# se-hwan/landing-controller

Hardware: AMD Instinct MI355X
Metric: landing NLPs solved/sec (SRBM, N=40, batch) (higher is better)
Workload: dtype f64

## Files before the change

### landing-controller_amd/csrc/solver_capi.inc

```

namespace {

struct StageTab {
  std::vector<int> tg_ab, tg_start, tg_term, gm_start, gm_term, a_term, r_start, r_term;
  int nu;
  std::vector<std::array<int, 4>> cterm;
  std::vector<std::array<int, 4>> rterm;
  std::vector<unsigned long long> cloc;
  bool operator==(const StageTab& o) const {
    return nu == o.nu && tg_ab == o.tg_ab && tg_start == o.tg_start && tg_term == o.tg_term && gm_start == o.gm_start &&
           gm_term == o.gm_term && a_term == o.a_term && r_start == o.r_start && r_term == o.r_term && cloc == o.cloc;
  }
};

int w_index(const Layout& L, int k, long long c) {
  const int N = L.N;
  if (c >= L.x_X(k) && c < L.x_X(k) + 12) return (int)(c - L.x_X(k));
  if (c >= L.x_U(k) && c < L.x_U(k) + 24) { const int j = (int)(c - L.x_U(k)); return j < 12 ? 12 + j : 24 + (j - 12); }
  if (k < N - 1 && c >= L.x_U(k + 1) && c < L.x_U(k + 1) + 12) return 36 + (int)(c - L.x_U(k + 1));
  return -1;
}
int jpos(const Layout& L, int k, long long c, long long idx) {
  if (c >= L.x_X(k) && c < L.x_X(k) + 12) return landing::NZ_JX + (int)(idx - L.jx(k));
  if (c >= L.x_U(k) && c < L.x_U(k) + 24) return landing::NZ_JU + (int)(idx - L.ju(k));
// ... 353 lines not shown
  if (!(o.theta_mu > 0.0)) o.theta_mu = ctx->L.run_cost ? 1.5 : 1.8;
  if (!(o.mu_init > 0.0)) o.mu_init = ctx->L.run_cost ? 0.1 : 0.5;
  if (!(o.bound_push > 0.0)) o.bound_push = ctx->L.run_cost ? 0.5 : 1.0;
  std::lock_guard<std::mutex> lock(ctx->mu);
  const int rc = ctx->ws.ensure(ctx->L, B, (hipStream_t)stream);
  if (rc) return fail(rc <= -100 ? LANDING_E_HIP : LANDING_E_ARG, "landing_solve_batch: workspace/table setup failed (" + std::to_string(rc) + ")");
  landing::SolveArgs A;
  A.L = ctx->L; A.B = B; A.o = o; A.p = d_p; A.x0 = d_x0; A.x_out = d_x; A.f_out = d_f; A.lam_out = d_lam_g;
  A.status = d_status; A.iters = d_iters; A.kkt = d_kkt; A.ws = ctx->ws.buf.get(); A.ws_stride = landing::member_stride(ctx->L);
  A.ctab = ctx->ws.d_ctab.get(); A.ctype = ctx->ws.d_ctype.get(); A.c_ml = ctx->ws.c_ml; A.c_mid = ctx->ws.c_mid; A.ccomb = ctx->ws.d_ccomb.get();
  A.rterm = (const unsigned long long*)ctx->ws.d_rterm.get(); A.rlen = ctx->ws.rlen;
  A.prof = ctx->d_prof;
  A.edge_map = ctx->d_edge_map.get();
  A.order = nullptr;
  if (o.dispatch_order && B > 512 && B <= 16384) {
    hipLaunchKernelGGL(landing::landing_order_kernel, dim3((B + 255) / 256), dim3(256), 0, (hipStream_t)stream, ctx->L, B, d_p, ctx->ws.d_order.get());
    A.order = ctx->ws.d_order.get();
  }
  hipLaunchKernelGGL(landing::landing_ipm_kernel, dim3(B), dim3(landing::SOLVER_THREADS), 0, (hipStream_t)stream, A);
  HIP_TRY(hipGetLastError());
  HIP_TRY(hipEventRecord(ctx->ws.done, (hipStream_t)stream));
  return 0;
}

int landing_set_profile_buffer(landing_ctx* ctx, double* d_prof) {
  if (!ctx) return fail(LANDING_E_ARG, "landing_set_profile_buffer: bad argument");
  ctx->d_prof = d_prof;
  return 0;
}

int landing_solve_batch_host(landing_ctx* ctx, int B, const double* p, const double* x0, const landing_solver_opts* opts,
// ... 516 lines not shown
```

### landing-controller_amd/csrc/solver_kernels.hip

```cpp
#include <hip/hip_runtime.h>
#include <math.h>

#include "../../include/landing_nlp.h"
#include "ipm_core.hpp"


namespace landing {

constexpr int NZ_JX = 0, NZ_JU = 157, NZ_JUN = 385, NZ_HX = 613, NZ_HU = 642, NZ_HUN = 802, NZ_TOT = 962;
constexpr int GS = 49;
constexpr int PS = 25;
constexpr int YS = 37;
constexpr int RIC_K = 0, RIC_KAP = 576, RIC_MT = 600, RIC_MV = 888, RIC_PX = 900, RIC_PV = 1188, RIC_STRIDE = 1200;
constexpr int RIC_FWD0 = 288, RIC_FWDN = 612;
constexpr int FILT_CAP = 64;
constexpr int SOLVER_NMAX = 96;
constexpr int ES = 26;
constexpr int SOLVER_THREADS = 256;
constexpr int COND_GAM = 480, COND_AH = 528, COND_STRIDE = 704;
constexpr int RCG = 36;
constexpr int RUNC = 48;

constexpr int CTAB_MLMAX = 6;
__host__ __device__ inline unsigned long long cterm_pack(int sa, int oa, int sb, int ob, bool has_b, int rowq, int rtype, int dst, bool closes) {
  const int nz[7] = {NZ_JX, NZ_JU, NZ_JUN, NZ_HX, NZ_HU, NZ_HUN, NZ_TOT};
  const unsigned pa = (unsigned)(nz[sa] + oa), pb = (unsigned)(nz[sb] + ob);
  const unsigned lo = pa | (pb << 11) | ((unsigned)(has_b ? 1 : 0) << 22) | ((unsigned)rowq << 23) | ((unsigned)rtype << 30);
  const unsigned hi = (unsigned)dst | ((unsigned)(closes ? 1 : 0) << 10);
  return (unsigned long long)lo | ((unsigned long long)hi << 32);
}
__host__ __device__ inline bool cterm_closes(unsigned long long t) { return ((t >> 42) & 1ull) != 0; }
constexpr int CX_SR = NZ_TOT + 48, CX_ONE = CX_SR + 208, CX_MONE = CX_ONE + 1, CX_ZERO = CX_ONE + 2, CX_LEN = CX_ONE + 3;
constexpr int ATAB_TB = 6, ATAB_LTMAX = 6;
constexpr int ASM_NSLOT = 512;

inline size_t member_stride(const Layout& L) {
  return (size_t)4 * L.nx + (size_t)14 * L.ng + L.nnz_jac + L.nnz_hess + (size_t)L.N * RUNC + (size_t)(L.N + 1) * RIC_STRIDE + (size_t)L.N * RCG;
}

enum { PH_EVAL = 0, PH_ERR, PH_SIGRHO, PH_BACK, PH_FWD, PH_DUAL, PH_LS, PH_ACCEPT, PH_NFACT, PH_NTRIAL, PH_NITER, PH_NSTAGE_OK, PH_B_ASM, PH_NSTAGE, PH_B_ELIM, PH_B_POST,
       PH_COUNT = 16 };
#define PROF_ADD(slot, tstart) do { if (SH.prof_on) { const long long n_ = (long long)wall_clock64(); if (threadIdx.x == 0) { SH.prof[slot] += (double)(n_ - (tstart)); (tstart) = n_; } } } while (0)

struct SolveArgs {
  Layout L; int B; landing_solver_opts o; double* prof;
  const double* p; const double* x0;
  double* x_out; double* f_out; double* lam_out; int* status; int* iters; double* kkt;
  double* ws; size_t ws_stride;
  const unsigned long long* rterm; int rlen;
  const unsigned long long* ctab; const int* ctype; int c_ml, c_mid;
  const unsigned long long* ccomb;
  const int* edge_map;
  const int* order;
};

struct MemberMem {
  double *x, *xt, *dx, *gx;
  double *g, *gt, *s, *ds, *zL, *zU, *y, *yn, *sig, *rho;
  double *J, *H, *Hc, *ric, *cond;
  double *en, *ep, *wn, *wp;
};

__device__ __forceinline__ MemberMem carve(const Layout& L, double* w) {
  MemberMem M;
  M.x = w; w += L.nx; M.xt = w; w += L.nx; M.dx = w; w += L.nx; M.gx = w; w += L.nx;
  M.g = w; w += L.ng; M.gt = w; w += L.ng; M.s = w; w += L.ng; M.ds = w; w += L.ng;
  M.zL = w; w += L.ng; M.zU = w; w += L.ng;
  M.y = w; w += L.ng; M.yn = w; w += L.ng;
  M.sig = w; w += L.ng; M.rho = w; w += L.ng;
  M.J = w; w += L.nnz_jac; M.H = w; w += L.nnz_hess; M.Hc = w; w += (size_t)L.N * RUNC; M.ric = w; w += (size_t)(L.N + 1) * RIC_STRIDE; M.cond = w; w += (size_t)L.N * RCG;
  M.en = w; w += L.ng; M.ep = w; w += L.ng; M.wn = w; w += L.ng; M.wp = w;
  return M;
}


constexpr int FWD_DXL_NMAX = 64;
constexpr int XCH = 112 * 4;
static_assert(2 * XCH >= 24 * YS, "A1 also holds Y (24 x YS)");
struct Lds {
  double G[48 * GS];
  double P[24 * PS];
  double A1[2 * XCH];
  double Ah[2 * 12 * YS];
  double gam[48], pv[24], q[24], bv[2 * 12], sig[24], w[48], dinv[24];
  double red[(SOLVER_THREADS / 64) * 6];
  double filt_th[FILT_CAP], filt_ph[FILT_CAP];
  double prof[32];
  int flag;
  int segb[SOLVER_NMAX * 8];
  double carry[ASM_NSLOT];
  double rcl[RCG];
  double jhl[CX_LEN];
  double dump[64];
  const unsigned long long* ctab; const unsigned long long* ccomb; int c_ml, c_mid, rc_on;
  double bnd_lb[36 + 2 * 104], bnd_ub[36 + 2 * 104];
  MemberMem M; Layout L; const double* p; int prof_on;
  IpmCtl ks;
  int clip_now, jamrun, action, fact_failed;
  unsigned long long atab_mid[ATAB_LTMAX * SOLVER_THREADS];
  unsigned long long acomb_mid[SOLVER_THREADS];
};
__shared__ Lds SH;
static_assert(36 * FWD_DXL_NMAX + 12 <= 24 * PS + 2 * XCH + 2 * 12 * YS && offsetof(Lds, A1) == offsetof(Lds, P) + sizeof(double) * 24 * PS && offsetof(Lds, Ah) == offsetof(Lds, A1) + sizeof(double) * 2 * XCH,
              "dx (x layout, N <= FWD_DXL_NMAX) fits the adjacent arrays [P | A1 | A^] (forward_pass / row_products)");
static_assert(offsetof(Lds, atab_mid) <= 65528, "the assembly tables address G, A^, gamma, cx, the partial sums and the dump slots with 16-bit byte offsets");
__host__ __device__ inline unsigned long long aterm_pack(int pa, int pb, int pc, int d, bool keep, bool ah) {
  const unsigned lo = (unsigned)pa | ((unsigned)pb << 16);
  const unsigned hi = (unsigned)pc | (((unsigned)d | (keep ? 1u : 0u) | (ah ? 2u : 0u)) << 16);
  return (unsigned long long)lo | ((unsigned long long)hi << 32);
}
__host__ __device__ inline unsigned long long acomb_pack(int n, int s0, int d, bool ah) {
  return (unsigned long long)((unsigned)n | ((unsigned)s0 << 16)) | ((unsigned long long)((unsigned)d | (ah ? 2u : 0u)) << 32);
}

template <int KT, class FA, class FB>
__device__ __forceinline__ f64x4 mfma_tile(f64x4 c, FA fa, FB fb) {
  const int l = threadIdx.x & 63, ij = l & 15, kq = l >> 4;
// ... 333 lines not shown
template <int NU>
__device__ __forceinline__ bool riccati_step(double* rec, double delta, int k) {
  const bool ok = block_eliminate<NU>(rec, delta, k);
  __syncthreads();
  return ok;
}

__device__ __noinline__ bool riccati_backward(double delta) {
  Lds& S = SH;
  const Layout& L = S.L;
  const MemberMem& M = S.M;
  const double* p = S.p;
  const int N = L.N, lane = threadIdx.x, NT = blockDim.x;
  (void)p; (void)N; (void)lane; (void)NT;
  bool ok = true;
  for (int e = lane; e < 24 * PS; e += NT) S.P[e] = 0.0;
  __syncthreads();
  if (lane < 12) {
    const int i = lane;
    const int ra = i < 6 ? 12 + i : 24 + (i - 6), rb = i < 6 ? 18 + i : 30 + (i - 6);
    const double qn2 = S.ks.feas ? 0.0 : 2.0 * p[L.o_QN + i];
    S.P[i * PS + i] = qn2 + M.sig[ra] + M.sig[rb] + delta;
    S.pv[i] = qn2 * (M.x[12 * N + i] - p[12 * N + i]) + M.rho[ra] + M.rho[rb];
    double* rec = M.ric + (size_t)N * RIC_STRIDE;
    for (int j = 0; j < 24; ++j) rec[RIC_PX + i * 24 + j] = (j == i) ? S.P[i * PS + i] : 0.0;
    rec[RIC_PV + i] = S.pv[i];
  }
  for (int e = lane; e < 48 * GS; e += NT) S.G[e] = 0.0;
  for (int e = lane; e < 2 * 12 * YS; e += NT) S.Ah[e] = 0.0;
  if (lane < 24) S.pv[lane] = (lane < 12) ? S.pv[lane] : 0.0;
// ... 1 lines not shown
  {
    AsmRegs first;
    asm_issue(N - 1, first);
    asm_copy(first);
    __syncthreads();
    asm_terms(N - 1, (N - 1) & 1, first);
    __syncthreads();
    asm_combine(N - 1, (N - 1) & 1);
  }
  __syncthreads();
  for (int k = N - 1; k >= 0 && ok; --k) {
    const bool last = (k == N - 1);
    long long tb_ = S.prof_on ? (long long)wall_clock64() : 0;
    double* rec = M.ric + (size_t)k * RIC_STRIDE;
    ok = last ? riccati_step<12>(rec, delta, k) : riccati_step<24>(rec, delta, k);
    if (lane == 0) { S.prof[PH_NSTAGE] += 1.0; if (ok) S.prof[PH_NSTAGE_OK] += 1.0; }
    PROF_ADD(PH_B_ELIM, tb_);
  }
  if (ok) {
    if (lane < 12) {
      const int i = lane;
      const double x0i = (i < 6) ? p[L.o_q_init + i] : p[L.o_qd_init + i - 6];
      S.sig[i] = x0i - M.x[i];
    }
    for (int e = lane; e < 144; e += NT) { const int i = e / 12, j = e % 12; S.G[(24 + i) * GS + 24 + j] = S.P[(12 + i) * PS + 12 + j]; }
    __syncthreads();
    if (lane < 12) {
      double v = S.pv[12 + lane];
      for (int t = 0; t < 12; ++t) v += S.P[(12 + lane) * PS + t] * S.sig[t];
      S.gam[24 + lane] = v;
    }
    __syncthreads();
    if (lane < 64) gauss_jordan_wave<12>(S.G, S.gam, S.A1, S.A1 + 24 * 24, &S.flag);
    __syncthreads();
    ok = S.flag != 0;
    if (lane == 0) { S.prof[PH_NSTAGE] += 1.0; if (ok) S.prof[PH_NSTAGE_OK] += 1.0; }
    if (ok) {
      if (lane < 12) S.sig[12 + lane] = -S.A1[24 * 24 + lane];
      __syncthreads();
    }
  }
  __syncthreads();
  return ok;
}

__device__ __noinline__ void forward_pass() {
  Lds& S = SH;
  const Layout& L = S.L;
  const MemberMem& M = S.M;
  const int N = L.N, tid = threadIdx.x, NT = blockDim.x;
  double* sg = S.G;
  double* buf = S.jhl;
  double* buf1 = S.A1;
  static_assert(24 * (SOLVER_NMAX + 1) <= 48 * GS && RIC_FWDN <= NZ_TOT + RUNC && RIC_FWDN <= XCH * 2, "forward scratch fits");
  auto slot = [&](int k) { return (k & 1) ? buf1 : buf; };
  auto fetch = [&](int k, double (&r)[3]) {
// ... 155 lines not shown
__global__ void landing_mpc_shift_kernel(Layout L, int B, const double* __restrict__ x_prev, const double* __restrict__ state,
                                         double* __restrict__ p, double* __restrict__ x0) {
  const size_t idx = (size_t)blockIdx.x * blockDim.x + threadIdx.x;
  if (idx >= (size_t)B * L.nx) return;
  const int m = (int)(idx / L.nx), i = (int)(idx % L.nx), N = L.N, nX = 12 * (N + 1);
  const double* xp = x_prev + (size_t)m * L.nx;
  double v;
  if (i < 12) v = state[(size_t)m * 12 + i];
  else if (i < nX) { const int k = i / 12, r = i % 12; v = xp[12 * (k < N ? k + 1 : N) + r]; }
  else { const int j = i - nX, k = j / 24, r = j % 24; v = xp[nX + 24 * (k < N - 1 ? k + 1 : N - 1) + r]; }
  x0[idx] = v;
  if (i < 6) p[(size_t)m * L.np + L.o_q_init + i] = v;
  else if (i < 12) p[(size_t)m * L.np + L.o_qd_init + (i - 6)] = v;
}

__global__ void landing_order_kernel(Layout L, int B, const double* __restrict__ p, int* __restrict__ order) {
  const int m = blockIdx.x * blockDim.x + threadIdx.x;
  if (m >= B) return;
  const int off = L.o_q_init + 2;
  double key = p[(size_t)m * L.np + off];
  if (!(key == key)) key = -INFINITY;
  int rank = 0;
  for (int j = 0; j < B; ++j) {
    double kj = p[(size_t)j * L.np + off];
    if (!(kj == kj)) kj = -INFINITY;
    rank += (kj > key) || (kj == key && j < m);
  }
  order[rank] = m;
}

__global__ void __launch_bounds__(SOLVER_THREADS, SOLVER_MIN_WAVES) landing_ipm_kernel(SolveArgs A) {
  if ((int)blockIdx.x >= A.B) return;
  const int m = A.order ? A.order[blockIdx.x] : (int)blockIdx.x;
  const Layout& L = A.L;
  const int N = L.N, lane = threadIdx.x, NT = blockDim.x;
  const int nx = L.nx, ng = L.ng;
  const double* p = A.p + (size_t)m * L.np;
  const landing_solver_opts& o = A.o;
  const MemberMem M = carve(L, A.ws + (size_t)m * A.ws_stride);
  Lds& S = SH;
  const double INF = INFINITY;
  auto bidx = [N](int r) { if (r < 36) return r; const int k = (r - 36) / 104, q = (r - 36) - 104 * k; return 36 + (k == N - 1 ? 104 : 0) + q; };
  double* __restrict__ r_g = M.g; double* __restrict__ r_gt = M.gt; double* __restrict__ r_s = M.s; double* __restrict__ r_ds = M.ds;
  double* __restrict__ r_zL = M.zL; double* __restrict__ r_zU = M.zU;
  double* __restrict__ r_y = M.y; double* __restrict__ r_yn = M.yn; double* __restrict__ r_sig = M.sig; double* __restrict__ r_rho = M.rho;
  S.M = M; S.L = L; S.p = p; S.prof_on = A.prof != nullptr;
  S.ctab = A.ctab; S.ccomb = A.ccomb; S.c_ml = A.c_ml; S.c_mid = A.c_mid; S.rc_on = 0;
  if (lane < SOLVER_THREADS) S.acomb_mid[lane] = A.ccomb[A.c_mid * SOLVER_THREADS + lane];
  for (int e = lane; e < 64; e += NT) S.dump[e] = 0.0;
  for (int e = lane; e < A.c_ml * SOLVER_THREADS; e += NT) S.atab_mid[e] = A.ctab[(size_t)A.c_mid * A.c_ml * SOLVER_THREADS + e];
  if (lane == 0) { S.jhl[CX_ONE] = 1.0; S.jhl[CX_MONE] = -1.0; S.jhl[CX_ZERO] = 0.0; }
  if (lane < 32) S.prof[lane] = 0.0;
  {
    const int nj = L.nnz_jac, nh = L.nnz_hess;
    for (int k = lane; k < N; k += NT) {
      int* sb = S.segb + k * 8;
      sb[0] = L.jx(k); sb[1] = L.ju(k); sb[2] = k < N - 1 ? L.ju(k + 1) : 0;
      sb[3] = nj + L.hx(k); sb[4] = nj + L.hu(k); sb[5] = k < N - 1 ? nj + L.hu(k + 1) : 0;
      sb[6] = nj + nh + k * RUNC; sb[7] = A.ctype[k];
    }
  }
  __syncthreads();

  for (int i = lane; i < nx; i += NT) {
    double v = A.x0[(size_t)m * nx + i];
    if (i < 6) v = p[L.o_q_init + i]; else if (i < 12) v = p[L.o_qd_init + i - 6];
    M.x[i] = v;
  }
  for (int e = lane; e < 36 + 2 * 104; e += NT) {
    const int r = e < 36 ? e : (e < 36 + 104 ? L.g_stage(0) + (e - 36) : L.g_stage(N - 1) + (e - 36 - 104));
    double lb = 0.0, ub = 0.0;
    if (r < ng) bound_of(L, p, r, lb, ub);
    S.bnd_lb[e] = lb; S.bnd_ub[e] = ub;
  }
  __syncthreads();
  if (L.run_cost) rc_init_hc();
  __syncthreads();
  member_eval_g_rare(L, M.x, p, M.g);
  __syncthreads();
  auto init_slacks = [&](bool back, double mu_) {
    for (int r = lane; r < ng; r += NT) { const double lb = S.bnd_lb[bidx(r)], ub = S.bnd_ub[bidx(r)]; ipm_init_row(M, r, r >= 12 && lb != ub, lb, ub, o, back, mu_); }
    __syncthreads();
  };
  init_slacks(false, 0.0);
  IpmCtl& K = S.ks;
#define KS_BEGIN() __syncthreads(); if (lane == 0) {
#define KS_BEGIN_SYNCED() if (lane == 0) {
#define KS_END() } __syncthreads()
  constexpr int RB = 4;
  auto feas_point_pass = [&](double mu_) {
    ElAcc e{};
    for (int r = lane; r < ng; r += NT) {
      double sg = 0.0, rh = 0.0;
      if (r >= 12) el_point_row(e, M, r, S.bnd_lb[bidx(r)], S.bnd_ub[bidx(r)], mu_, o.feas_rho, sg, rh);
      r_sig[r] = sg; r_rho[r] = rh;
    }
    el_point_finish(K, e, S.red);
  };
  auto point_pass = [&](double mu_) {
    if (K.feas) { feas_point_pass(mu_); return; }
    double pr = 0.0, co = 0.0, cm = 0.0, ys = 0.0, zs = 0.0, nz = 0.0;
    for (int rb = lane; rb < ng; rb += NT * RB) {
      double lbv[RB], ubv[RB], gv[RB], sv[RB], zlv[RB], zuv[RB], yv[RB];
#pragma unroll
      for (int j = 0; j < RB; ++j) { const int r = rb + j * NT, rr = r < ng ? r : ng - 1; lbv[j] = S.bnd_lb[bidx(rr)]; ubv[j] = S.bnd_ub[bidx(rr)]; gv[j] = r_g[rr]; sv[j] = r_s[rr]; zlv[j] = r_zL[rr]; zuv[j] = r_zU[rr]; yv[j] = r_y[rr]; }
#pragma unroll
      for (int j = 0; j < RB; ++j) {
        const int r = rb + j * NT;
        if (r >= ng) continue;
        const double lb = lbv[j], ub = ubv[j];
        double sg = 0.0, rh = 0.0;
        if (r >= 12) {
          const double g = gv[j];
          ys += fabs(yv[j]);
          if (lb == ub) pr = fmax(pr, fabs(g - lb));
// ... 4 lines not shown
            if (ub < INF) { const double d = ub - s, rd = fast_rcp(d), zu = zuv[j]; co = fmax(co, d * zu); cm = fmax(cm, fabs(d * zu - mu_)); sg += zu * rd; rh += mu_ * rd; zs += zu; nz += 1.0; }
            rh += sg * (g - s);
          }
        }
        r_sig[r] = sg; r_rho[r] = rh;
      }
    }
    double v[6] = {pr, co, cm, ys, zs, nz}; const int op[6] = {RMAX, RMAX, RMAX, RSUM, RSUM, RSUM};
    block_reduce<6>(v, op, S.red);
    KS_BEGIN_SYNCED() K.c_pr = v[0]; K.c_co = v[1]; K.c_cm = v[2]; K.c_ys = v[3]; K.c_zs = v[4]; K.c_nz = fmax(v[5], 1.0); KS_END();
  };

  if (lane == 0) {
    ipm_init(K, o);
    K.tp = A.prof ? (long long)wall_clock64() : 0;
    S.clip_now = 0; S.jamrun = 0; S.fact_failed = 0;
  }
  __syncthreads();
  const int nst = N > 36 ? N : 36;

  for (;;) {
    if (A.prof && lane == 0) K.tp = (long long)wall_clock64();
    if ((lane & 63) < nst) member_eval_jh(L, M.x, p, M.y, M.J, M.H, M.gx, nullptr, nullptr, K.feas ? 0.0 : 1.0);
    __syncthreads();
    if (L.run_cost && !K.feas) { rc_add_grad(); __syncthreads(); }
    PROF_ADD(PH_EVAL, K.tp);
    if (K.it == 0) point_pass(K.mu);
    {
      double du = 0.0;
      for (int i = lane + 12; i < nx; i += NT) du = fmax(du, fabs(M.gx[i]));
      du = block_reduce1(du, RMAX, S.red);
      KS_BEGIN_SYNCED()
        ipm_errors(K, o, du);
        S.action = ipm_decide(K, o, S.fact_failed != 0);
        S.fact_failed = 0;
      KS_END();
// ... 64 lines not shown
      if (!K.flag) break;
    }
    if (!K.fact_ok) {
      KS_BEGIN() K.status = K.stalled ? LANDING_STALLED : LANDING_NUMERICAL; S.fact_failed = (o.feas_phase && !K.feas_used && !K.feas) ? 1 : 0; KS_END();
      if (S.fact_failed) continue;
      break;
    }
    KS_BEGIN() ipm_commit_delta(K, o, 0.0); KS_END();
    PROF_ADD(PH_BACK, K.tp);

    forward_pass();
    row_products(A.rterm, A.rlen);

    PROF_ADD(PH_FWD, K.tp);
    {
      const double mu = K.mu;
      const bool feas = K.feas != 0;
      const bool clip_now = !feas && K.clip_k_cur > 1 && (K.c_pr > o.clip_until || (o.jam_clip > 0 && S.jamrun >= o.jam_clip));
      double top[4] = {0.0, 0.0, 0.0, 0.0};
      double m_pr = 0.0, m_du = 0.0, th0 = 0.0, bar = 0.0, dphi = 0.0;
      double f0 = 0.0;
      if (feas) {
        const double frho = o.feas_rho;
        for (int r = lane + 12; r < ng; r += NT) {
          const double lb = S.bnd_lb[bidx(r)], ub = S.bnd_ub[bidx(r)], g = r_g[r];
          if (lb == ub) { th0 += fabs(g - lb); continue; }
          const double s = r_s[r];
          double ds = r_ds[r];
          if (r >= 36) { ds = ds + (g - s); r_ds[r] = ds; }
          th0 += fabs(g - s);
// ... 51 lines not shown
      block_reduce<6>(v, op, S.red);
      if (clip_now) block_top4(top, S.red);
      KS_BEGIN_SYNCED()
        const double tau = K.tau;
        double a_pr = (v[0] > tau) ? tau / v[0] : 1.0;
        K.a_du = (v[1] > tau) ? tau / v[1] : 1.0;
        if (clip_now) {
          const double rk = top[(K.clip_k_cur > 4 ? 4 : K.clip_k_cur) - 1];
          a_pr = (rk > tau) ? tau / rk : 1.0;
        }
        K.a_pr = a_pr;
        S.clip_now = clip_now ? 1 : 0; K.omt = clip_now ? 1.0 - tau : -1.0;
        K.th0 = v[2]; K.dphi = v[4]; K.ph0 = v[5] + mu * v[3];
        if (K.th_max == 0.0) K.th_max = 1e4 * fmax(1.0, v[2]);
        K.alpha = a_pr; K.s_corr = 0.0; K.accepted = 0; K.armijo_step = 0; K.ls_done = a_pr > 1e-10 ? 0 : 1;
      KS_END();
    }
    PROF_ADD(PH_DUAL, K.tp);
    while (!K.ls_done) {
      const double alpha = K.alpha, omt = K.omt, mu = K.mu;
      if (lane == 0) S.prof[PH_NTRIAL] += 1.0;
      for (int i = lane; i < nx; i += NT) M.xt[i] = M.x[i] + alpha * M.dx[i];
      __syncthreads();
      if (lane < nst) member_eval_g(L, M.xt, p, M.gt);
      __syncthreads();
      double tht = 0.0, bt = 0.0, ft = 0.0;
      const bool feas = K.feas != 0;
      if (feas) {
        const double frho = o.feas_rho;
        for (int r = lane + 12; r < ng; r += NT) {
          const double lb = S.bnd_lb[bidx(r)], ub = S.bnd_ub[bidx(r)], g = r_gt[r];
          if (lb == ub) { tht += fabs(g - lb); continue; }
          const double s0 = r_s[r], ds = r_ds[r], s = s0 + alpha * ds;
          tht += fabs(g - s);
          if (lb > -INF) { const double n0 = M.en[r]; const ElStep e = el_step(1.0, s0 - lb + n0, n0, r_zL[r], M.wn[r], mu, frho, ds); const double n = n0 + alpha * e.dn; bt -= log((s - lb + n) * n); ft += frho * n; }
          if (ub < INF) { const double q0 = M.ep[r]; const ElStep e = el_step(-1.0, ub + q0 - s0, q0, r_zU[r], M.wp[r], mu, frho, ds); const double q = q0 + alpha * e.dn; bt -= log((ub + q - s) * q); ft += frho * q; }
        }
      } else
      for (int rb = lane + 12; rb < ng; rb += NT * RB) {
        double lbv[RB], ubv[RB], gv[RB], sv[RB], dsv[RB];
#pragma unroll
        for (int j = 0; j < RB; ++j) { const int r = rb + j * NT, rr = r < ng ? r : ng - 1; lbv[j] = S.bnd_lb[bidx(rr)]; ubv[j] = S.bnd_ub[bidx(rr)]; gv[j] = r_gt[rr]; sv[j] = r_s[rr]; dsv[j] = r_ds[rr]; }
#pragma unroll
        for (int j = 0; j < RB; ++j) {
          if (rb + j * NT >= ng) continue;
          const double lb = lbv[j], ub = ubv[j], g = gv[j];
          if (lb == ub) { tht += fabs(g - lb); continue; }
          double s = sv[j] + alpha * dsv[j];
          if (omt > 0.0) { if (lb > -INF) s = fmax(s, fma(omt, sv[j] - lb, lb)); if (ub < INF) s = fmin(s, fma(-omt, ub - sv[j], ub)); }
          tht += fabs(g - s);
          bt -= log((lb > -INF ? s - lb : 1.0) * (ub < INF ? ub - s : 1.0));
        }
      }
      if (lane < 12 && !feas) { const double d = M.xt[12 * N + lane] - p[12 * N + lane]; ft = p[L.o_QN + lane] * d * d; }
      if (L.run_cost && !feas) ft += rc_f(M.xt);
      { double v[3] = {tht, bt, ft}; const int op[3] = {RSUM, RSUM, RSUM}; block_reduce<3>(v, op, S.red); tht = v[0]; bt = v[1]; ft = v[2]; }
      KS_BEGIN_SYNCED() ipm_ls_test(K, o, tht, ft, bt, S.filt_th, S.filt_ph); KS_END();
      if (K.need_corr) {
        double tht2 = 0.0, bt2 = 0.0;
        for (int rb = lane + 12; rb < ng; rb += NT * RB) {
          double lbv[RB], ubv[RB], gv[RB], sv[RB], dsv[RB];
#pragma unroll
          for (int j = 0; j < RB; ++j) { const int r = rb + j * NT, rr = r < ng ? r : ng - 1; lbv[j] = S.bnd_lb[bidx(rr)]; ubv[j] = S.bnd_ub[bidx(rr)]; gv[j] = r_gt[rr]; sv[j] = r_s[rr]; dsv[j] = r_ds[rr]; }
#pragma unroll
          for (int j = 0; j < RB; ++j) {
            if (rb + j * NT >= ng) continue;
            const double lb = lbv[j], ub = ubv[j], g = gv[j];
            if (lb == ub) { tht2 += fabs(g - lb); continue; }
            double s = sv[j] + alpha * dsv[j];
            if (omt > 0.0) { if (lb > -INF) s = fmax(s, fma(omt, sv[j] - lb, lb)); if (ub < INF) s = fmin(s, fma(-omt, ub - sv[j], ub)); }
            const double lo = lb > -INF ? lb + o.slack_corr * (s - lb) : -INF, hi = ub < INF ? ub - o.slack_corr * (ub - s) : INF;
            s = fmin(fmax(g, lo), hi);
            tht2 += fabs(g - s);
            bt2 -= log((lb > -INF ? s - lb : 1.0) * (ub < INF ? ub - s : 1.0));
          }
        }
        { double v[2] = {tht2, bt2}; const int op[2] = {RSUM, RSUM}; block_reduce<2>(v, op, S.red); tht2 = v[0]; bt2 = v[1]; }
        KS_BEGIN_SYNCED() ipm_ls_corr_test(K, o, tht2, bt2, S.filt_th, S.filt_ph); KS_END();
      }
    }
    KS_BEGIN()
      ipm_ls_end(K, o, S.filt_th, S.filt_ph, FILT_CAP);
      if (o.jam_clip > 0) S.jamrun = (!S.clip_now && K.a_pr < 0.02) ? S.jamrun + 1 : 0;
    KS_END();
    if (K.fallback) {
      const double alpha = K.alpha;
      for (int i = lane; i < nx; i += NT) M.xt[i] = M.x[i] + alpha * M.dx[i];
      __syncthreads();
      member_eval_g_rare(L, M.xt, p, M.gt);
      __syncthreads();
    }
    PROF_ADD(PH_LS, K.tp);
    for (int i = lane; i < nx; i += NT) M.x[i] = M.xt[i];
    if (K.feas) {
      const double alpha = K.alpha, a_du = K.a_du, mu = K.mu, frho = o.feas_rho;
      for (int r = lane; r < ng; r += NT) {
        const double lb = S.bnd_lb[bidx(r)], ub = S.bnd_ub[bidx(r)];
        r_g[r] = r_gt[r];
        if (r < 12) continue;
// ... 6 lines not shown
          const double n = n0 + alpha * e.dn, a = s - lb + n;
          zl = fmin(fmax(z0 + a_du * e.dz, 1e-10 * mu / a), 1e10 * mu / a);
          M.wn[r] = fmin(fmax(w0 + a_du * e.dw, 1e-10 * mu / n), 1e10 * mu / n); M.en[r] = n;
        }
        if (ub < INF) {
          const double q0 = M.ep[r], z0 = r_zU[r], w0 = M.wp[r];
          const ElStep e = el_step(-1.0, ub + q0 - s0, q0, z0, w0, mu, frho, ds);
          const double q = q0 + alpha * e.dn, b = ub + q - s;
          zu = fmin(fmax(z0 + a_du * e.dz, 1e-10 * mu / b), 1e10 * mu / b);
          M.wp[r] = fmin(fmax(w0 + a_du * e.dw, 1e-10 * mu / q), 1e10 * mu / q); M.ep[r] = q;
        }
        r_s[r] = s; r_zL[r] = zl; r_zU[r] = zu; r_y[r] = zu - zl;
      }
      __syncthreads();
      feas_point_pass(mu);
      KS_BEGIN() K.it++; KS_END();
    } else {
      const double alpha = K.alpha, a_du = K.a_du, omt = K.omt, mu = K.mu, s_corr = K.s_corr;
      double npr = 0.0, nco = 0.0, ncm = 0.0, nys = 0.0, nzs = 0.0, nnz = 0.0;
      for (int rb = lane; rb < ng; rb += NT * RB) {
        double lbv[RB], ubv[RB], gv[RB], sv[RB], dsv[RB], zlv[RB], zuv[RB], yv[RB], ynv[RB];
#pragma unroll
        for (int j = 0; j < RB; ++j) {
          const int r = rb + j * NT, rr = r < ng ? r : ng - 1;
          lbv[j] = S.bnd_lb[bidx(rr)]; ubv[j] = S.bnd_ub[bidx(rr)]; gv[j] = r_gt[rr]; sv[j] = r_s[rr]; dsv[j] = r_ds[rr]; zlv[j] = r_zL[rr]; zuv[j] = r_zU[rr]; yv[j] = r_y[rr]; ynv[j] = r_yn[rr];
        }
#pragma unroll
        for (int j = 0; j < RB; ++j) {
          const int r = rb + j * NT;
          if (r >= ng) continue;
          const double lb = lbv[j], ub = ubv[j], g = gv[j];
// ... 21 lines not shown
                nco = fmax(nco, d * zu); ncm = fmax(ncm, fabs(d * zu - mu)); sg += zu * rd; rh += mu * rd; nzs += zu; nnz += 1.0;
              }
              npr = fmax(npr, fabs(g - s));
              rh += sg * (g - s);
              r_s[r] = s; r_zL[r] = zl; r_zU[r] = zu; r_y[r] = zu - zl; nys += fabs(zu - zl);
            }
          }
          r_sig[r] = sg; r_rho[r] = rh;
        }
      }
      double v[6] = {npr, nco, ncm, nys, nzs, nnz}; const int op[6] = {RMAX, RMAX, RMAX, RSUM, RSUM, RSUM};
      block_reduce<6>(v, op, S.red);
      KS_BEGIN_SYNCED()
        K.c_pr = v[0]; K.c_co = v[1]; K.c_cm = v[2]; K.c_ys = v[3]; K.c_zs = v[4]; K.c_nz = fmax(v[5], 1.0);
        K.it++;
      KS_END();
    }
    PROF_ADD(PH_ACCEPT, K.tp);
  }
  __syncthreads();
  if (A.prof && lane == 0) { S.prof[PH_NITER] = (double)K.it; for (int i = 0; i < PH_COUNT; ++i) A.prof[(size_t)m * PH_COUNT + i] = S.prof[i]; }

  double fo = 0.0;
  if (lane < 12) { M.y[lane] = -M.gx[lane]; const double d = M.x[12 * N + lane] - p[12 * N + lane]; fo = p[L.o_QN + lane] * d * d; }
  if (L.run_cost) fo += rc_f(M.x);
  fo = block_reduce1(fo, RSUM, S.red);
  double kp = 0.0, kc = 0.0;
  for (int r = lane; r < ng; r += NT) {
    const double lb = S.bnd_lb[bidx(r)], ub = S.bnd_ub[bidx(r)], g = M.g[r], lam = M.y[r];
    kp = fmax(kp, fmax(lb - g, fmax(g - ub, 0.0)));
    if (lb != ub) {
      const double dist = lam > 0.0 ? ub - g : g - lb;
      if (lam != 0.0 && dist < INF) kc = fmax(kc, fabs(lam * dist));
    }
  }
  { double v[2] = {kp, kc}; const int op[2] = {RMAX, RMAX}; block_reduce<2>(v, op, S.red); kp = v[0]; kc = v[1]; }
  for (int i = lane; i < nx; i += NT) A.x_out[(size_t)m * nx + i] = M.x[i];
  if (A.lam_out) for (int r = lane; r < ng; r += NT) A.lam_out[(size_t)m * ng + r] = M.y[r];
  if (lane == 0) {
    if (A.f_out) A.f_out[m] = fo;
    if (A.status) A.status[m] = K.status;
    if (A.iters) A.iters[m] = K.it;
    if (A.kkt) { A.kkt[3 * m] = kp; A.kkt[3 * m + 1] = K.e_du; A.kkt[3 * m + 2] = kc; }
  }
#undef KS_BEGIN
#undef KS_BEGIN_SYNCED
#undef KS_END
}

}
```

Measured before the change: 19910.

## Fuse first line-search trial with acceptance pass via double-buffered row arrays

On the first line-search trial of a non-feasibility iteration, the kernel now computes the accepted slacks, duals, sigma and rho into a second set of row buffers together with the trial merit terms. It folds the convergence norms into a single 9-value block reduction. When the trial is accepted, pointers are swapped (including x/xt and g/gt) and the separate acceptance pass is skipped, removing a full row sweep and its barriers. In exchange it adds six more per-row workspace arrays, per-phase pointer reloads from shared memory via readfirstlane, and extra work when the first trial is rejected. It also rewrites the order kernel to stage keys through shared memory in tiles and batches the profiling counters for stage attempts.

```diff
diff --git a/landing-controller_amd/csrc/solver_capi.inc b/landing-controller_amd/csrc/solver_capi.inc
--- a/landing-controller_amd/csrc/solver_capi.inc
+++ b/landing-controller_amd/csrc/solver_capi.inc
@@ -391,7 +391,7 @@
   A.edge_map = ctx->d_edge_map.get();
   A.order = nullptr;
   if (o.dispatch_order && B > 512 && B <= 16384) {
-    hipLaunchKernelGGL(landing::landing_order_kernel, dim3((B + 255) / 256), dim3(256), 0, (hipStream_t)stream, ctx->L, B, d_p, ctx->ws.d_order.get());
+    hipLaunchKernelGGL(landing::landing_order_kernel, dim3((B + landing::ORDER_THREADS - 1) / landing::ORDER_THREADS), dim3(landing::ORDER_THREADS), 0, (hipStream_t)stream, ctx->L, B, d_p, ctx->ws.d_order.get());
     A.order = ctx->ws.d_order.get();
   }
   hipLaunchKernelGGL(landing::landing_ipm_kernel, dim3(B), dim3(landing::SOLVER_THREADS), 0, (hipStream_t)stream, A);
diff --git a/landing-controller_amd/csrc/solver_kernels.hip b/landing-controller_amd/csrc/solver_kernels.hip
--- a/landing-controller_amd/csrc/solver_kernels.hip
+++ b/landing-controller_amd/csrc/solver_kernels.hip
@@ -1,5 +1,6 @@
 #include <hip/hip_runtime.h>
 #include <math.h>
+#include <type_traits>
 
 #include "../../include/landing_nlp.h"
 #include "ipm_core.hpp"
@@ -35,12 +36,30 @@
 constexpr int ASM_NSLOT = 512;
 
 inline size_t member_stride(const Layout& L) {
-  return (size_t)4 * L.nx + (size_t)14 * L.ng + L.nnz_jac + L.nnz_hess + (size_t)L.N * RUNC + (size_t)(L.N + 1) * RIC_STRIDE + (size_t)L.N * RCG;
+  return (size_t)4 * L.nx + (size_t)20 * L.ng + L.nnz_jac + L.nnz_hess + (size_t)L.N * RUNC + (size_t)(L.N + 1) * RIC_STRIDE + (size_t)L.N * RCG;
 }
 
 enum { PH_EVAL = 0, PH_ERR, PH_SIGRHO, PH_BACK, PH_FWD, PH_DUAL, PH_LS, PH_ACCEPT, PH_NFACT, PH_NTRIAL, PH_NITER, PH_NSTAGE_OK, PH_B_ASM, PH_NSTAGE, PH_B_ELIM, PH_B_POST,
        PH_COUNT = 16 };
 #define PROF_ADD(slot, tstart) do { if (SH.prof_on) { const long long n_ = (long long)wall_clock64(); if (threadIdx.x == 0) { SH.prof[slot] += (double)(n_ - (tstart)); (tstart) = n_; } } } while (0)
+
+enum { EMU_ACC_FAST = 0, EMU_ACC_FAST_CLIP, EMU_ACC_FIRST_REJECTED, EMU_ACC_BACKTRACK, EMU_ACC_CORR, EMU_ACC_FALLBACK, EMU_ACC_FEAS, EMU_ACC_N };
+#ifndef __HIPCC__
+constexpr int EMU_ACC_MAXB = 64;
+static int emu_acc[EMU_ACC_MAXB][EMU_ACC_N];
+#define LANDING_EMU_COUNT(m, what) do { if ((m) < EMU_ACC_MAXB) emu_acc[m][what]++; } while (0)
+static int emu_fused_on = 1;
+#define LANDING_EMU_FUSED_ON (emu_fused_on != 0)
+extern "C" void landing_emu_set_fused(int on) { emu_fused_on = on; }
+extern "C" int landing_emu_accept_counts(int m, int* counts) {
+  if (m < 0 || m >= EMU_ACC_MAXB || !counts) return -1;
+  for (int i = 0; i < EMU_ACC_N; ++i) counts[i] = emu_acc[m][i];
+  return 0;
+}
+#else
+#define LANDING_EMU_COUNT(m, what) ((void)0)
+#define LANDING_EMU_FUSED_ON true
+#endif
 
 struct SolveArgs {
   Layout L; int B; landing_solver_opts o; double* prof;
@@ -59,7 +78,11 @@
   double *g, *gt, *s, *ds, *zL, *zU, *y, *yn, *sig, *rho;
   double *J, *H, *Hc, *ric, *cond;
   double *en, *ep, *wn, *wp;
+  double *sig2, *rho2, *s2, *zL2, *zU2, *y2;
 };
+constexpr int MEMBER_MEM_PTRS = 29;
+static_assert(sizeof(MemberMem) == MEMBER_MEM_PTRS * sizeof(double*) && std::is_standard_layout<MemberMem>::value && std::is_trivially_copyable<MemberMem>::value,
+              "live_mem() walks MemberMem as an array of double*: nothing but double* members");
 
 __device__ __forceinline__ MemberMem carve(const Layout& L, double* w) {
   MemberMem M;
@@ -69,8 +92,18 @@
   M.y = w; w += L.ng; M.yn = w; w += L.ng;
   M.sig = w; w += L.ng; M.rho = w; w += L.ng;
   M.J = w; w += L.nnz_jac; M.H = w; w += L.nnz_hess; M.Hc = w; w += (size_t)L.N * RUNC; M.ric = w; w += (size_t)(L.N + 1) * RIC_STRIDE; M.cond = w; w += (size_t)L.N * RCG;
-  M.en = w; w += L.ng; M.ep = w; w += L.ng; M.wn = w; w += L.ng; M.wp = w;
+  M.en = w; w += L.ng; M.ep = w; w += L.ng; M.wn = w; w += L.ng; M.wp = w; w += L.ng;
+  M.sig2 = w; w += L.ng; M.rho2 = w; w += L.ng;
+  M.s2 = w; w += L.ng; M.zL2 = w; w += L.ng; M.zU2 = w; w += L.ng; M.y2 = w;
   return M;
+}
+
+__host__ __device__ __forceinline__ void mem_accept_swap(MemberMem& M) {
+  double* t;
+#define LANDING_SWAP(a, b) t = M.a; M.a = M.b; M.b = t
+  LANDING_SWAP(s, s2); LANDING_SWAP(zL, zL2); LANDING_SWAP(zU, zU2); LANDING_SWAP(y, y2); LANDING_SWAP(sig, sig2); LANDING_SWAP(rho, rho2);
+  LANDING_SWAP(g, gt); LANDING_SWAP(x, xt);
+#undef LANDING_SWAP
 }
 
 
@@ -83,7 +116,7 @@
   double A1[2 * XCH];
   double Ah[2 * 12 * YS];
   double gam[48], pv[24], q[24], bv[2 * 12], sig[24], w[48], dinv[24];
-  double red[(SOLVER_THREADS / 64) * 6];
+  double red[(SOLVER_THREADS / 64) * 9];
   double filt_th[FILT_CAP], filt_ph[FILT_CAP];
   double prof[32];
   int flag;
@@ -97,10 +130,25 @@
   MemberMem M; Layout L; const double* p; int prof_on;
   IpmCtl ks;
   int clip_now, jamrun, action, fact_failed;
+  int first_trial, fast;
+  double nxt[6];
   unsigned long long atab_mid[ATAB_LTMAX * SOLVER_THREADS];
   unsigned long long acomb_mid[SOLVER_THREADS];
 };
 __shared__ Lds SH;
+__device__ __forceinline__ MemberMem live_mem() {
+  MemberMem M = SH.M;
+#if defined(__HIP_DEVICE_COMPILE__)
+  double** q = reinterpret_cast<double**>(&M);
+#pragma unroll
+  for (int i = 0; i < MEMBER_MEM_PTRS; ++i) {
+    const unsigned long long a = (unsigned long long)q[i];
+    const unsigned lo = (unsigned)__builtin_amdgcn_readfirstlane((int)(unsigned)a), hi = (unsigned)__builtin_amdgcn_readfirstlane((int)(unsigned)(a >> 32));
+    q[i] = (double*)((unsigned long long)lo | ((unsigned long long)hi << 32));
+  }
+#endif
+  return M;
+}
 static_assert(36 * FWD_DXL_NMAX + 12 <= 24 * PS + 2 * XCH + 2 * 12 * YS && offsetof(Lds, A1) == offsetof(Lds, P) + sizeof(double) * 24 * PS && offsetof(Lds, Ah) == offsetof(Lds, A1) + sizeof(double) * 2 * XCH,
               "dx (x layout, N <= FWD_DXL_NMAX) fits the adjacent arrays [P | A1 | A^] (forward_pass / row_products)");
 static_assert(offsetof(Lds, atab_mid) <= 65528, "the assembly tables address G, A^, gamma, cx, the partial sums and the dump slots with 16-bit byte offsets");
@@ -464,6 +512,7 @@
   const int N = L.N, lane = threadIdx.x, NT = blockDim.x;
   (void)p; (void)N; (void)lane; (void)NT;
   bool ok = true;
+  int n_try = 0;
   for (int e = lane; e < 24 * PS; e += NT) S.P[e] = 0.0;
   __syncthreads();
   if (lane < 12) {
@@ -495,7 +544,7 @@
     long long tb_ = S.prof_on ? (long long)wall_clock64() : 0;
     double* rec = M.ric + (size_t)k * RIC_STRIDE;
     ok = last ? riccati_step<12>(rec, delta, k) : riccati_step<24>(rec, delta, k);
-    if (lane == 0) { S.prof[PH_NSTAGE] += 1.0; if (ok) S.prof[PH_NSTAGE_OK] += 1.0; }
+    ++n_try;
     PROF_ADD(PH_B_ELIM, tb_);
   }
   if (ok) {
@@ -515,12 +564,13 @@
     if (lane < 64) gauss_jordan_wave<12>(S.G, S.gam, S.A1, S.A1 + 24 * 24, &S.flag);
     __syncthreads();
     ok = S.flag != 0;
-    if (lane == 0) { S.prof[PH_NSTAGE] += 1.0; if (ok) S.prof[PH_NSTAGE_OK] += 1.0; }
+    ++n_try;
     if (ok) {
       if (lane < 12) S.sig[12 + lane] = -S.A1[24 * 24 + lane];
       __syncthreads();
     }
   }
+  if (lane == 0) { S.prof[PH_NSTAGE] += (double)n_try; S.prof[PH_NSTAGE_OK] += (double)(ok ? n_try : n_try - 1); }
   __syncthreads();
   return ok;
 }
@@ -706,19 +756,24 @@
   else if (i < 12) p[(size_t)m * L.np + L.o_qd_init + (i - 6)] = v;
 }
 
-__global__ void landing_order_kernel(Layout L, int B, const double* __restrict__ p, int* __restrict__ order) {
-  const int m = blockIdx.x * blockDim.x + threadIdx.x;
-  if (m >= B) return;
+constexpr int ORDER_THREADS = 256;
+__global__ void __launch_bounds__(ORDER_THREADS) landing_order_kernel(Layout L, int B, const double* __restrict__ p, int* __restrict__ order) {
+  __shared__ double keys[ORDER_THREADS];
+  const int tid = threadIdx.x, m = blockIdx.x * ORDER_THREADS + tid;
   const int off = L.o_q_init + 2;
-  double key = p[(size_t)m * L.np + off];
+  double key = m < B ? p[(size_t)m * L.np + off] : 0.0;
   if (!(key == key)) key = -INFINITY;
   int rank = 0;
-  for (int j = 0; j < B; ++j) {
-    double kj = p[(size_t)j * L.np + off];
+  for (int j0 = 0; j0 < B; j0 += ORDER_THREADS) {
+    double kj = j0 + tid < B ? p[(size_t)(j0 + tid) * L.np + off] : 0.0;
     if (!(kj == kj)) kj = -INFINITY;
-    rank += (kj > key) || (kj == key && j < m);
-  }
-  order[rank] = m;
+    keys[tid] = kj;
+    __syncthreads();
+    const int n = B - j0 < ORDER_THREADS ? B - j0 : ORDER_THREADS;
+    for (int j = 0; j < n; ++j) rank += (keys[j] > key) || (keys[j] == key && j0 + j < m);
+    __syncthreads();
+  }
+  if (m < B) order[rank] = m;
 }
 
 __global__ void __launch_bounds__(SOLVER_THREADS, SOLVER_MIN_WAVES) landing_ipm_kernel(SolveArgs A) {
@@ -733,9 +788,10 @@
   Lds& S = SH;
   const double INF = INFINITY;
   auto bidx = [N](int r) { if (r < 36) return r; const int k = (r - 36) / 104, q = (r - 36) - 104 * k; return 36 + (k == N - 1 ? 104 : 0) + q; };
-  double* __restrict__ r_g = M.g; double* __restrict__ r_gt = M.gt; double* __restrict__ r_s = M.s; double* __restrict__ r_ds = M.ds;
-  double* __restrict__ r_zL = M.zL; double* __restrict__ r_zU = M.zU;
-  double* __restrict__ r_y = M.y; double* __restrict__ r_yn = M.yn; double* __restrict__ r_sig = M.sig; double* __restrict__ r_rho = M.rho;
+#define ROW_PTRS(M) double* __restrict__ r_g = (M).g; double* __restrict__ r_gt = (M).gt; double* __restrict__ r_s = (M).s; double* __restrict__ r_ds = (M).ds; \
+  double* __restrict__ r_zL = (M).zL; double* __restrict__ r_zU = (M).zU; double* __restrict__ r_y = (M).y; double* __restrict__ r_yn = (M).yn; \
+  double* __restrict__ r_sig = (M).sig; double* __restrict__ r_rho = (M).rho; \
+  (void)r_g; (void)r_gt; (void)r_s; (void)r_ds; (void)r_zL; (void)r_zU; (void)r_y; (void)r_yn; (void)r_sig; (void)r_rho
   S.M = M; S.L = L; S.p = p; S.prof_on = A.prof != nullptr;
   S.ctab = A.ctab; S.ccomb = A.ccomb; S.c_ml = A.c_ml; S.c_mid = A.c_mid; S.rc_on = 0;
   if (lane < SOLVER_THREADS) S.acomb_mid[lane] = A.ccomb[A.c_mid * SOLVER_THREADS + lane];
@@ -743,6 +799,9 @@
   for (int e = lane; e < A.c_ml * SOLVER_THREADS; e += NT) S.atab_mid[e] = A.ctab[(size_t)A.c_mid * A.c_ml * SOLVER_THREADS + e];
   if (lane == 0) { S.jhl[CX_ONE] = 1.0; S.jhl[CX_MONE] = -1.0; S.jhl[CX_ZERO] = 0.0; }
   if (lane < 32) S.prof[lane] = 0.0;
+#ifndef __HIPCC__
+  if (lane == 0 && m < EMU_ACC_MAXB) for (int i = 0; i < EMU_ACC_N; ++i) emu_acc[m][i] = 0;
+#endif
   {
     const int nj = L.nnz_jac, nh = L.nnz_hess;
     for (int k = lane; k < N; k += NT) {
@@ -771,16 +830,20 @@
   member_eval_g_rare(L, M.x, p, M.g);
   __syncthreads();
   auto init_slacks = [&](bool back, double mu_) {
+    const MemberMem M = live_mem();
     for (int r = lane; r < ng; r += NT) { const double lb = S.bnd_lb[bidx(r)], ub = S.bnd_ub[bidx(r)]; ipm_init_row(M, r, r >= 12 && lb != ub, lb, ub, o, back, mu_); }
     __syncthreads();
   };
   init_slacks(false, 0.0);
+  for (int r = lane; r < ng; r += NT) { M.s2[r] = 0.0; M.zL2[r] = 0.0; M.zU2[r] = 0.0; M.y2[r] = 0.0; M.sig2[r] = 0.0; M.rho2[r] = 0.0; }
   IpmCtl& K = S.ks;
 #define KS_BEGIN() __syncthreads(); if (lane == 0) {
 #define KS_BEGIN_SYNCED() if (lane == 0) {
 #define KS_END() } __syncthreads()
   constexpr int RB = 4;
   auto feas_point_pass = [&](double mu_) {
+    const MemberMem M = live_mem();
+    ROW_PTRS(M);
     ElAcc e{};
     for (int r = lane; r < ng; r += NT) {
       double sg = 0.0, rh = 0.0;
@@ -791,6 +854,8 @@
   };
   auto point_pass = [&](double mu_) {
     if (K.feas) { feas_point_pass(mu_); return; }
+    const MemberMem M = live_mem();
+    ROW_PTRS(M);
     double pr = 0.0, co = 0.0, cm = 0.0, ys = 0.0, zs = 0.0, nz = 0.0;
     for (int rb = lane; rb < ng; rb += NT * RB) {
       double lbv[RB], ubv[RB], gv[RB], sv[RB], zlv[RB], zuv[RB], yv[RB];
@@ -825,12 +890,13 @@
   if (lane == 0) {
     ipm_init(K, o);
     K.tp = A.prof ? (long long)wall_clock64() : 0;
-    S.clip_now = 0; S.jamrun = 0; S.fact_failed = 0;
+    S.clip_now = 0; S.jamrun = 0; S.fact_failed = 0; S.first_trial = 0; S.fast = 0;
   }
   __syncthreads();
   const int nst = N > 36 ? N : 36;
 
   for (;;) {
+    const MemberMem M = live_mem();
     if (A.prof && lane == 0) K.tp = (long long)wall_clock64();
     if ((lane & 63) < nst) member_eval_jh(L, M.x, p, M.y, M.J, M.H, M.gx, nullptr, nullptr, K.feas ? 0.0 : 1.0);
     __syncthreads();
@@ -925,6 +991,8 @@
 
     PROF_ADD(PH_FWD, K.tp);
     {
+      const MemberMem M = live_mem();
+      ROW_PTRS(M);
       const double mu = K.mu;
       const bool feas = K.feas != 0;
       const bool clip_now = !feas && K.clip_k_cur > 1 && (K.c_pr > o.clip_until || (o.jam_clip > 0 && S.jamrun >= o.jam_clip));
@@ -1006,17 +1074,22 @@
         K.th0 = v[2]; K.dphi = v[4]; K.ph0 = v[5] + mu * v[3];
         if (K.th_max == 0.0) K.th_max = 1e4 * fmax(1.0, v[2]);
         K.alpha = a_pr; K.s_corr = 0.0; K.accepted = 0; K.armijo_step = 0; K.ls_done = a_pr > 1e-10 ? 0 : 1;
+        S.first_trial = (feas || !LANDING_EMU_FUSED_ON) ? 0 : 1; S.fast = 0;
       KS_END();
     }
     PROF_ADD(PH_DUAL, K.tp);
     while (!K.ls_done) {
+      const MemberMem M = live_mem();
+      ROW_PTRS(M);
       const double alpha = K.alpha, omt = K.omt, mu = K.mu;
+      const bool fused = S.first_trial != 0;
       if (lane == 0) S.prof[PH_NTRIAL] += 1.0;
       for (int i = lane; i < nx; i += NT) M.xt[i] = M.x[i] + alpha * M.dx[i];
       __syncthreads();
       if (lane < nst) member_eval_g(L, M.xt, p, M.gt);
       __syncthreads();
       double tht = 0.0, bt = 0.0, ft = 0.0;
+      double npr = 0.0, nco = 0.0, ncm = 0.0, nys = 0.0, nzs = 0.0, nnz = 0.0;
       const bool feas = K.feas != 0;
       if (feas) {
         const double frho = o.feas_rho;
@@ -1028,6 +1101,54 @@
           if (lb > -INF) { const double n0 = M.en[r]; const ElStep e = el_step(1.0, s0 - lb + n0, n0, r_zL[r], M.wn[r], mu, frho, ds); const double n = n0 + alpha * e.dn; bt -= log((s - lb + n) * n); ft += frho * n; }
           if (ub < INF) { const double q0 = M.ep[r]; const ElStep e = el_step(-1.0, ub + q0 - s0, q0, r_zU[r], M.wp[r], mu, frho, ds); const double q = q0 + alpha * e.dn; bt -= log((ub + q - s) * q); ft += frho * q; }
         }
+      } else if (fused) {
+        const double a_du = o.dual_step_cap > 0.0 ? fmin(K.a_du, o.dual_step_cap * alpha) : K.a_du;
+        double* __restrict__ w_s = M.s2; double* __restrict__ w_zL = M.zL2; double* __restrict__ w_zU = M.zU2; double* __restrict__ w_y = M.y2;
+        double* __restrict__ w_sig = M.sig2; double* __restrict__ w_rho = M.rho2;
+        for (int rb = lane + 12; rb < ng; rb += NT * RB) {
+          double lbv[RB], ubv[RB], gv[RB], sv[RB], dsv[RB], zlv[RB], zuv[RB], yv[RB], ynv[RB];
+#pragma unroll
+          for (int j = 0; j < RB; ++j) {
+            const int r = rb + j * NT, rr = r < ng ? r : ng - 1;
+            lbv[j] = S.bnd_lb[bidx(rr)]; ubv[j] = S.bnd_ub[bidx(rr)]; gv[j] = r_gt[rr]; sv[j] = r_s[rr]; dsv[j] = r_ds[rr]; zlv[j] = r_zL[rr]; zuv[j] = r_zU[rr]; yv[j] = r_y[rr]; ynv[j] = r_yn[rr];
+          }
+#pragma unroll
+          for (int j = 0; j < RB; ++j) {
+            const int r = rb + j * NT;
+            if (r >= ng) continue;
+            const double lb = lbv[j], ub = ubv[j], g = gv[j];
+            double sg = 0.0, rh = 0.0;
+            if (lb == ub) {
+              tht += fabs(g - lb);
+              const double yn_ = yv[j] + alpha * (ynv[j] - yv[j]); w_y[r] = yn_; nys += fabs(yn_); npr = fmax(npr, fabs(g - lb));
+            } else {
+              const double so = sv[j], ds = dsv[j];
+              double s = so + alpha * ds;
+              if (omt > 0.0) { if (lb > -INF) s = fmax(s, fma(omt, so - lb, lb)); if (ub < INF) s = fmin(s, fma(-omt, ub - so, ub)); }
+              tht += fabs(g - s);
+              bt -= log((lb > -INF ? s - lb : 1.0) * (ub < INF ? ub - s : 1.0));
+              double zl = 0.0, zu = 0.0;
+              if (lb > -INF) {
+                const double dold = so - lb, ro = fast_rcp(dold), zo = zlv[j], dz = fma(-zo * ro, ds, mu * ro - zo), d = s - lb, rd = fast_rcp(d);
+                zl = fmin(fmax(zo + a_du * dz, 1e-10 * mu * rd), 1e10 * mu * rd);
+                nco = fmax(nco, d * zl); ncm = fmax(ncm, fabs(d * zl - mu)); sg += zl * rd; rh -= mu * rd; nzs += zl; nnz += 1.0;
+              }
+              if (ub < INF) {
+                const double dold = ub - so, ro = fast_rcp(dold), zo = zuv[j], dz = fma(zo * ro, ds, mu * ro - zo), d = ub - s, rd = fast_rcp(d);
+                zu = fmin(fmax(zo + a_du * dz, 1e-10 * mu * rd), 1e10 * mu * rd);
+                nco = fmax(nco, d * zu); ncm = fmax(ncm, fabs(d * zu - mu)); sg += zu * rd; rh += mu * rd; nzs += zu; nnz += 1.0;
+              }
+              npr = fmax(npr, fabs(g - s));
+              rh += sg * (g - s);
+              w_s[r] = s; w_zL[r] = zl; w_zU[r] = zu; w_y[r] = zu - zl; nys += fabs(zu - zl);
+            }
+            w_sig[r] = sg; w_rho[r] = rh;
+          }
+        }
+        static_assert(ASM_NSLOT >= 2 * SOLVER_THREADS, "carry takes two partial sums per thread");
+        { const int t = lane + 12 < NT ? lane + 12 : lane + 12 - NT; S.carry[2 * t] = nys; S.carry[2 * t + 1] = nzs; }
+        __syncthreads();
+        nys = S.carry[2 * lane]; nzs = S.carry[2 * lane + 1];
       } else
       for (int rb = lane + 12; rb < ng; rb += NT * RB) {
         double lbv[RB], ubv[RB], gv[RB], sv[RB], dsv[RB];
@@ -1046,8 +1167,19 @@
       }
       if (lane < 12 && !feas) { const double d = M.xt[12 * N + lane] - p[12 * N + lane]; ft = p[L.o_QN + lane] * d * d; }
       if (L.run_cost && !feas) ft += rc_f(M.xt);
-      { double v[3] = {tht, bt, ft}; const int op[3] = {RSUM, RSUM, RSUM}; block_reduce<3>(v, op, S.red); tht = v[0]; bt = v[1]; ft = v[2]; }
-      KS_BEGIN_SYNCED() ipm_ls_test(K, o, tht, ft, bt, S.filt_th, S.filt_ph); KS_END();
+      if (fused) {
+        double v[9] = {tht, bt, ft, npr, nco, ncm, nys, nzs, nnz}; const int op[9] = {RSUM, RSUM, RSUM, RMAX, RMAX, RMAX, RSUM, RSUM, RSUM};
+        block_reduce<9>(v, op, S.red);
+        KS_BEGIN_SYNCED()
+          ipm_ls_test(K, o, v[0], v[2], v[1], S.filt_th, S.filt_ph);
+          S.first_trial = 0; S.fast = K.accepted;
+          for (int i = 0; i < 6; ++i) S.nxt[i] = v[3 + i];
+          LANDING_EMU_COUNT(m, K.accepted ? (omt > 0.0 ? EMU_ACC_FAST_CLIP : EMU_ACC_FAST) : EMU_ACC_FIRST_REJECTED);
+        KS_END();
+      } else {
+        { double v[3] = {tht, bt, ft}; const int op[3] = {RSUM, RSUM, RSUM}; block_reduce<3>(v, op, S.red); tht = v[0]; bt = v[1]; ft = v[2]; }
+        KS_BEGIN_SYNCED() ipm_ls_test(K, o, tht, ft, bt, S.filt_th, S.filt_ph); KS_END();
+      }
       if (K.need_corr) {
         double tht2 = 0.0, bt2 = 0.0;
         for (int rb = lane + 12; rb < ng; rb += NT * RB) {
@@ -1074,7 +1206,25 @@
     KS_BEGIN()
       ipm_ls_end(K, o, S.filt_th, S.filt_ph, FILT_CAP);
       if (o.jam_clip > 0) S.jamrun = (!S.clip_now && K.a_pr < 0.02) ? S.jamrun + 1 : 0;
+      if (S.fast) {
+#ifndef __HIPCC__
+        for (int r = 0; r < ng; ++r) {
+          const MemberMem& Q = S.M;
+          const bool eq = r >= 12 && S.bnd_lb[bidx(r)] == S.bnd_ub[bidx(r)];
+          if ((r < 12 && (Q.y[r] != Q.y2[r] || Q.sig[r] != Q.sig2[r] || Q.rho[r] != Q.rho2[r])) || (eq && (Q.s[r] != Q.s2[r] || Q.zL[r] != Q.zL2[r] || Q.zU[r] != Q.zU2[r]))) {
+            fprintf(stderr, "landing_ipm_kernel: member %d row %d differs between the two instances of the row arrays at a swap\n", m, r); abort();
+          }
+        }
+#endif
+        mem_accept_swap(S.M);
+        K.c_pr = S.nxt[0]; K.c_co = S.nxt[1]; K.c_cm = S.nxt[2]; K.c_ys = S.nxt[3]; K.c_zs = S.nxt[4]; K.c_nz = fmax(S.nxt[5], 1.0);
+        K.it++;
+      }
     KS_END();
+    if (S.fast) { PROF_ADD(PH_LS, K.tp); PROF_ADD(PH_ACCEPT, K.tp); continue; }
+    {
+    const MemberMem M = live_mem();
+    ROW_PTRS(M);
     if (K.fallback) {
       const double alpha = K.alpha;
       for (int i = lane; i < nx; i += NT) M.xt[i] = M.x[i] + alpha * M.dx[i];
@@ -1111,7 +1261,7 @@
       }
       __syncthreads();
       feas_point_pass(mu);
-      KS_BEGIN() K.it++; KS_END();
+      KS_BEGIN() K.it++; LANDING_EMU_COUNT(m, EMU_ACC_FEAS); KS_END();
     } else {
       const double alpha = K.alpha, a_du = K.a_du, omt = K.omt, mu = K.mu, s_corr = K.s_corr;
       double npr = 0.0, nco = 0.0, ncm = 0.0, nys = 0.0, nzs = 0.0, nnz = 0.0;
@@ -1163,13 +1313,17 @@
       KS_BEGIN_SYNCED()
         K.c_pr = v[0]; K.c_co = v[1]; K.c_cm = v[2]; K.c_ys = v[3]; K.c_zs = v[4]; K.c_nz = fmax(v[5], 1.0);
         K.it++;
+        LANDING_EMU_COUNT(m, K.fallback ? EMU_ACC_FALLBACK : (s_corr > 0.0 ? EMU_ACC_CORR : EMU_ACC_BACKTRACK));
       KS_END();
     }
     PROF_ADD(PH_ACCEPT, K.tp);
+    }
   }
   __syncthreads();
   if (A.prof && lane == 0) { S.prof[PH_NITER] = (double)K.it; for (int i = 0; i < PH_COUNT; ++i) A.prof[(size_t)m * PH_COUNT + i] = S.prof[i]; }
 
+  {
+  const MemberMem M = live_mem();
   double fo = 0.0;
   if (lane < 12) { M.y[lane] = -M.gx[lane]; const double d = M.x[12 * N + lane] - p[12 * N + lane]; fo = p[L.o_QN + lane] * d * d; }
   if (L.run_cost) fo += rc_f(M.x);
@@ -1192,6 +1346,8 @@
     if (A.iters) A.iters[m] = K.it;
     if (A.kkt) { A.kkt[3 * m] = kp; A.kkt[3 * m + 1] = K.e_du; A.kkt[3 * m + 2] = kc; }
   }
+  }
+#undef ROW_PTRS
 #undef KS_BEGIN
 #undef KS_BEGIN_SYNCED
 #undef KS_END
```

Measured after the change: 20220, median of 6. +1.5%, better.
